# oi-taa/rag-fin

Hardware: AMD Instinct MI355X
Metric: queries/sec, brute-force cosine/IP top-10 over a 1,000,000 x 384-d fp16 corpus, batch=64 (recall@10 vs CPU oracle reported alongside) (higher is better)
Workload: dtype f16; 1 GPU; 1M x 384-d fp16 corpus, batch-64 queries, top-10; rows_per_gpu=1000000, rows_total=1000000, dim=384, batch=64, topk=10, batches_in_flight=4, collective=none

## Files before the change

rag_fin_amd/csrc/api.hip:

```cpp
#include "rf_internal.h"
#include <stdlib.h>
#include <string.h>

struct rf_arena {
  unsigned char* base;
  size_t off;
  template <class T>
  T* take(size_t count) {
    T* p = base ? (T*)(base + off) : nullptr;
    off = (off + count * sizeof(T) + 255) / 256 * 256;
    return p;
  }
};

static rf_workspace carve(rf_arena& a) {
  rf_workspace ws;
  ws.thr = a.take<float>(RF_QWIDE);
  ws.eps = a.take<float>(RF_QWIDE);
  ws.cand_cnt = a.take<uint32_t>((size_t)RF_QWIDE * RF_CAND_SHARDS);
  ws.pmax = a.take<float>((size_t)RF_QWIDE * RF_SAMPLE_WGS);
  ws.cand = a.take<uint2>((size_t)RF_QWIDE * RF_CAND_SHARDS * RF_SHARD_CAP);
  ws.fold = a.take<uint4>((size_t)RF_FOLD_WAVES * RF_QCHUNK);
  ws.rmask = a.take<unsigned long long>(RF_FOLD_WAVES);
  ws.rlist = a.take<uint32_t>(RF_FOLD_BLOCKS);
// ... 82 lines not shown
static int check_search_args(const char* fn, const rf_index_t* ix, const void* q, int B, int k,
                             const void* scores, const void* ids, const void* ws, size_t ws_bytes) {
  if (!ix || !q || !scores || !ids || !ws) {
    rf_set_error("%s: null argument", fn);
    return RF_ERR_INVALID;
  }
  if (B <= 0) {
    rf_set_error("%s: B = %d", fn, B);
    return RF_ERR_INVALID;
  }
  if (k <= 0 || k > RF_MAX_K) {
    rf_set_error("%s: k = %d outside 1..%d", fn, k, RF_MAX_K);
    return RF_ERR_UNSUPPORTED;
  }
  if ((((uintptr_t)q) & 15) || (((uintptr_t)ws) & 15)) {
    rf_set_error("%s: q / workspace must be 16-byte aligned", fn);
    return RF_ERR_INVALID;
  }
  if (ws_bytes < rf_search_workspace_bytes(nullptr)) {
    rf_set_error("%s: workspace %zu B < required %zu B", fn, ws_bytes,
                 rf_search_workspace_bytes(nullptr));
    return RF_ERR_CAPACITY;
  }
  return RF_OK;
}

static int check_sq8(const char* fn, const rf_index_t* ix, size_t ws_bytes) {
  if (!ix->sq8_tiles) {
    rf_set_error("%s: no SQ8 shadow attached (rf_index_attach_sq8)", fn);
    return RF_ERR_INVALID;
  }
  if (ws_bytes < rf_search_sq8_workspace_bytes(ix)) {
    rf_set_error("%s: workspace %zu B < required %zu B", fn, ws_bytes, rf_search_sq8_workspace_bytes(ix));
    return RF_ERR_CAPACITY;
  }
  return RF_OK;
}

static int check_filter_arg(const char* fn, const void* filter_dev) {
  if (!filter_dev || (((uintptr_t)filter_dev) & 15)) {
    rf_set_error("%s: filter buffer null or not 16-byte aligned", fn);
    return RF_ERR_INVALID;
  }
  return RF_OK;
}

__global__ void k_fill_empty(int n, int B, float* scores, int64_t* ids, double* exact,
                             uint32_t* flags) {
  const int i = blockIdx.x * blockDim.x + threadIdx.x;
  if (i < n) {
    scores[i] = -INFINITY;
    ids[i] = -1;
    if (exact) exact[i] = -INFINITY;
  }
  if (flags && i < B) flags[i] = 0u;
}

struct rf_out {
  float* scores;
  int64_t* ids;
  double* exact;
  uint32_t* flags;
};

static int fill_empty(int B, int k, const rf_out& o, hipStream_t st) {
  const int n = B * k;
  hipLaunchKernelGGL(k_fill_empty, dim3((n + 255) / 256), dim3(256), 0, st, n, B, o.scores, o.ids,
                     o.exact, o.flags);
  RF_HIP(hipGetLastError());
  return RF_OK;
}

static bool take_wide(const rf_index_t* ix, int left, int k) {
  return rf_wide_supported(ix) && left > RF_QCHUNK && ix->size > RF_SMALL_ROWS && k <= 16 &&
         ix->size >= (int64_t)k * 1024;
}

static int chunk_width(const rf_index_t* ix, int left, int k, bool widen, bool* wide) {
  *wide = widen && take_wide(ix, left, k);
  const int cap = *wide ? RF_QWIDE : RF_QCHUNK;
  return left < cap ? left : cap;
}

template <class T>
static T* at(T* p, size_t off) { return p ? p + off : nullptr; }

template <class F>
static int for_chunks(const rf_index_t* ix, const void* q_dev, int B, int k, size_t row, bool widen,
                      const rf_out& o, F&& body) {
  for (int q0 = 0; q0 < B;) {
    bool wide;
    const int nb = chunk_width(ix, B - q0, k, widen, &wide);
    const size_t r0 = (size_t)q0 * row;
    const int rc = body(q0, nb, wide, (const _Float16*)q_dev + (size_t)q0 * ix->dim,
                        rf_out{at(o.scores, r0), at(o.ids, r0), at(o.exact, r0), at(o.flags, (size_t)q0)});
    if (rc != RF_OK) return rc;
    q0 += nb;
  }
  return RF_OK;
}

struct rf_variant {
  const rf_filter_view* filt;
  const rf_sq8_ws* sq8;
  bool wide;
  const rf_band* band;
  const rf_after* after;
  const rf_multi* multi;
  bool coarse;
};

static int mark(hipEvent_t* ev, int* n, hipStream_t st) {
  if (ev) RF_HIP(hipEventRecord(ev[(*n)++], st));
  return RF_OK;
}

template <class F>
static int time_stages(int marks, float* stage_ms, F run) {
  hipEvent_t ev[7];
  for (int i = 0; i < marks; ++i) RF_HIP(hipEventCreate(&ev[i]));
  const int rc = run(ev);
  if (rc == RF_OK) {
    RF_HIP(hipEventSynchronize(ev[marks - 1]));
    for (int i = 0; i + 1 < marks; ++i) RF_HIP(hipEventElapsedTime(&stage_ms[i], ev[i], ev[i + 1]));
  }
  for (int i = 0; i < marks; ++i) (void)hipEventDestroy(ev[i]);
  return rc;
}

static int sweep(const rf_index_t* ix, const rf_variant& v, const _Float16* qc, int nb, int k, int64_t id_base,
                 const rf_workspace& ws, const rf_out& o, hipStream_t st, hipEvent_t* ev) {
  const int JB = nb <= 32 ? 1 : 2;
  int P = 0, n_ev = 0;
  rf_fold kept{};
  rf_fold* fold = (v.wide || v.sq8 || v.filt || v.band) ? nullptr : &kept;
  int rc = mark(ev, &n_ev, st);
  if (v.sq8) {
    if (rc == RF_OK) rc = rf_launch_sq8_queries(ix, qc, nb, *v.sq8, st);
    if (rc == RF_OK && !v.coarse) rc = mark(ev, &n_ev, st);
  }
  if (rc == RF_OK && ix->size > RF_SMALL_ROWS && v.band) rc = rf_launch_band_eps(ix, qc, nb, ws, st);
  if (rc == RF_OK && ix->size > RF_SMALL_ROWS)
    rc = v.wide ? rf_launch_wide_sample(ix, qc, nb, ws, &P, st)
                : rf_launch_sample(ix, qc, nb, JB, ws, &P, st, v.filt, fold, v.band, v.after, v.multi);
  if (rc == RF_OK) rc = mark(ev, &n_ev, st);
  if (rc == RF_OK) rc = rf_launch_threshold(ix, qc, nb, k, P, ws, st, fold, v.sq8, v.band);
  if (rc == RF_OK) rc = mark(ev, &n_ev, st);
  if (rc == RF_OK)
    rc = v.wide  ? rf_launch_wide_emit(ix, qc, nb, ws, st)
         : v.sq8 ? rf_launch_sq8_emit(ix, nb, JB, ws, *v.sq8, st)
                 : rf_launch_emit(ix, qc, nb, JB, ws, st, v.filt, fold, v.band, v.after, v.multi);
  if (v.sq8) {
    if (rc == RF_OK && !v.coarse) rc = mark(ev, &n_ev, st);
    if (rc == RF_OK) rc = rf_launch_shadow_refine(ix, qc, nb, k, ws, *v.sq8, st);
  }
  if (rc == RF_OK) rc = mark(ev, &n_ev, st);
  if (rc == RF_OK) rc = rf_launch_merge(ix, qc, nb, k, id_base, ws, o.scores, o.ids, o.exact, o.flags, st, v.band, v.after);
  if (rc == RF_OK) rc = mark(ev, &n_ev, st);
  return rc;
}

enum { RF_FP16 = 0, RF_SQ8 = 1, RF_SHADOW = 2 };
static int search_enqueue(const rf_index_t* ix, const void* q_dev, int B, int k, int64_t id_base, const rf_out& o,
                          void* workspace_dev, hipStream_t st, const rf_filter_view* filt, int sq8,
                          float* stage_ms = nullptr, const rf_band* band = nullptr,
                          const rf_after* after = nullptr, const rf_multi* multi = nullptr) {
  if (ix->size == 0) return fill_empty(B, k, o, st);
  rf_arena a{(unsigned char*)workspace_dev, 0};
  rf_workspace ws;
  const rf_sq8_ws sw = carve_sq8(a, &ws);
  const rf_sq8_ws* sq = sq8 != RF_FP16 && ix->size > RF_SMALL_ROWS ? &sw : nullptr;
  const bool coarse = sq8 == RF_SHADOW;
  const bool widen = !filt && !sq && !band;
  if (!stage_ms)
    return for_chunks(ix, q_dev, B, k, (size_t)k, widen, o,
                      [&](int q0, int nb, bool wide, const _Float16* qc, const rf_out& oc) {
                        const rf_after ac{after ? after->score + q0 : nullptr, after ? after->id + q0 : nullptr};
                        const rf_multi mc{multi ? multi->masks_t : nullptr, multi ? multi->qfilter + q0 : nullptr,
                                          multi ? multi->gp : 0u};
                        return sweep(ix, rf_variant{filt, sq, wide, band, after ? &ac : nullptr, multi ? &mc : nullptr, coarse},
                                     qc, nb, k, id_base, ws, oc, st, nullptr);
                      });
  bool wide;
  const int nb = chunk_width(ix, B, k, widen, &wide);
  return time_stages(sq && !coarse ? 7 : 5, stage_ms, [&](hipEvent_t* ev) {
    return sweep(ix, rf_variant{filt, sq, wide, band, after, multi, coarse}, (const _Float16*)q_dev, nb, k, id_base, ws,
                 o, st, ev);
  });
}

static int plain_chain(const rf_index_t* ix, int B) {
  return shadow_first(ix) && ix->size >= ix->shadow_min_rows && ix->size > RF_SMALL_ROWS && B <= RF_QCHUNK ? RF_SHADOW
                                                                                                          : RF_FP16;
}

extern "C" int rf_index_set_shadow_first(rf_index_t* ix, int64_t min_rows) {
  if (!ix) {
    rf_set_error("rf_index_set_shadow_first: null index");
    return RF_ERR_INVALID;
  }
  ix->shadow_min_rows = min_rows > 0 ? min_rows : 0;
  return RF_OK;
}

extern "C" int rf_search(const rf_index_t* ix, const void* q_dev, int B, int k, int64_t id_base,
                         float* scores_dev, int64_t* ids_dev, double* exact_dev,
                         uint32_t* flags_dev, void* workspace_dev, size_t workspace_bytes,
                         void* stream) {
  int rc = check_search_args("rf_search", ix, q_dev, B, k, scores_dev, ids_dev, workspace_dev,
                             workspace_bytes);
  if (rc == RF_OK && plain_chain(ix, B) == RF_SHADOW) rc = check_sq8("rf_search", ix, workspace_bytes);
  if (rc != RF_OK) return rc;
  return search_enqueue(ix, q_dev, B, k, id_base, rf_out{scores_dev, ids_dev, exact_dev, flags_dev}, workspace_dev,
                        (hipStream_t)stream, nullptr, plain_chain(ix, B));
}

extern "C" int rf_search_fp16(const rf_index_t* ix, const void* q_dev, int B, int k, int64_t id_base,
                              float* scores_dev, int64_t* ids_dev, double* exact_dev,
                              uint32_t* flags_dev, void* workspace_dev, size_t workspace_bytes,
                              void* stream) {
  int rc = check_search_args("rf_search_fp16", ix, q_dev, B, k, scores_dev, ids_dev, workspace_dev,
                             workspace_bytes);
  if (rc != RF_OK) return rc;
  return search_enqueue(ix, q_dev, B, k, id_base, rf_out{scores_dev, ids_dev, exact_dev, flags_dev}, workspace_dev,
                        (hipStream_t)stream, nullptr, RF_FP16);
}

extern "C" int rf_search_profile(const rf_index_t* ix, const void* q_dev, int B, int k,
                                 int64_t id_base, float* scores_dev, int64_t* ids_dev,
                                 double* exact_dev, uint32_t* flags_dev, void* workspace_dev,
                                 size_t workspace_bytes, void* stream, float* stage_ms_host) {
  int rc = check_search_args("rf_search_profile", ix, q_dev, B, k, scores_dev, ids_dev,
                             workspace_dev, workspace_bytes);
  if (rc == RF_OK && plain_chain(ix, B) == RF_SHADOW) rc = check_sq8("rf_search_profile", ix, workspace_bytes);
  if (rc != RF_OK) return rc;
  if (!stage_ms_host || ix->size == 0) {
    rf_set_error("rf_search_profile: null stage buffer or empty index");
    return RF_ERR_INVALID;
  }
  return search_enqueue(ix, q_dev, B, k, id_base, rf_out{scores_dev, ids_dev, exact_dev, flags_dev}, workspace_dev,
                        (hipStream_t)stream, nullptr, plain_chain(ix, B), stage_ms_host);
}

extern "C" int rf_search_sq8(const rf_index_t* ix, const void* q_dev, int B, int k, int64_t id_base,
                             float* scores_dev, int64_t* ids_dev, double* exact_dev, uint32_t* flags_dev,
                             void* workspace_dev, size_t workspace_bytes, void* stream) {
  int rc = check_search_args("rf_search_sq8", ix, q_dev, B, k, scores_dev, ids_dev, workspace_dev,
                             workspace_bytes);
  if (rc != RF_OK) return rc;
  rc = check_sq8("rf_search_sq8", ix, workspace_bytes);
  if (rc != RF_OK) return rc;
  return search_enqueue(ix, q_dev, B, k, id_base, rf_out{scores_dev, ids_dev, exact_dev, flags_dev}, workspace_dev,
                        (hipStream_t)stream, nullptr, RF_SQ8);
}

extern "C" int rf_search_sq8_profile(const rf_index_t* ix, const void* q_dev, int B, int k, int64_t id_base,
                                     float* scores_dev, int64_t* ids_dev, double* exact_dev, uint32_t* flags_dev,
                                     void* workspace_dev, size_t workspace_bytes, void* stream,
                                     float* stage_ms_host) {
  int rc = check_search_args("rf_search_sq8_profile", ix, q_dev, B, k, scores_dev, ids_dev, workspace_dev,
                             workspace_bytes);
  if (rc != RF_OK) return rc;
  rc = check_sq8("rf_search_sq8_profile", ix, workspace_bytes);
  if (rc != RF_OK) return rc;
  if (!stage_ms_host || ix->size <= RF_SMALL_ROWS) {
    rf_set_error("rf_search_sq8_profile: null stage buffer or a corpus of <= %d rows", RF_SMALL_ROWS);
    return RF_ERR_INVALID;
  }
  return search_enqueue(ix, q_dev, B, k, id_base, rf_out{scores_dev, ids_dev, exact_dev, flags_dev}, workspace_dev,
                        (hipStream_t)stream, nullptr, RF_SQ8, stage_ms_host);
}

extern "C" int rf_debug_scores_sq8(const rf_index_t* ix, const void* q_dev, int B, int64_t n, float* out_dev,
                                   float* delta_dev, void* workspace_dev, size_t workspace_bytes, void* stream) {
  if (!ix || !q_dev || !out_dev || !workspace_dev || B <= 0 || n <= 0 || n > ix->size) {
    rf_set_error("rf_debug_scores_sq8: bad argument");
    return RF_ERR_INVALID;
  }
  int rc = check_sq8("rf_debug_scores_sq8", ix, workspace_bytes);
  if (rc != RF_OK) return rc;
  hipStream_t st = (hipStream_t)stream;
  rf_arena a{(unsigned char*)workspace_dev, 0};
  const rf_sq8_ws sw = carve_sq8(a, nullptr);
  return for_chunks(ix, q_dev, B, 0, (size_t)n, false, rf_out{out_dev, nullptr, nullptr, nullptr},
                    [&](int q0, int nb, bool, const _Float16* qc, const rf_out& oc) {
                      const int rc = rf_launch_sq8_queries(ix, qc, nb, sw, st);
                      return rc != RF_OK ? rc : rf_launch_sq8_debug(ix, nb, n, sw, oc.scores, at(delta_dev, (size_t)q0), st);
                    });
}

static int exhaustive_impl(const char* fn, const rf_index_t* ix, const void* q_dev, int B, int k,
                           int64_t id_base, float* scores_dev, int64_t* ids_dev, double* exact_dev,
                           const double* after_s, const int64_t* after_r, void* workspace_dev,
                           size_t workspace_bytes, void* stream, const uint32_t* mask = nullptr,
                           const rf_band* band = nullptr) {
  int rc = check_search_args(fn, ix, q_dev, B, k, scores_dev, ids_dev, workspace_dev, workspace_bytes);
  if (rc != RF_OK) return rc;
  hipStream_t st = (hipStream_t)stream;
  const rf_out o{scores_dev, ids_dev, exact_dev, nullptr};
  if (ix->size == 0) return fill_empty(B, k, o, st);
  rf_arena a{(unsigned char*)workspace_dev, 0};
  const rf_workspace ws = carve(a);
  return for_chunks(ix, q_dev, B, k, (size_t)k, false, o,
                    [&](int q0, int nb, bool, const _Float16* qc, const rf_out& oc) {
                      return rf_launch_exhaustive(ix, qc, nb, k, id_base, ws, oc.scores, oc.ids, oc.exact,
                                                  at(after_s, (size_t)q0), at(after_r, (size_t)q0), st, mask, band);
                    });
// ... 339 lines not shown
```

rag_fin_amd/csrc/rf_internal.h:

```cpp
#pragma once
#include <hip/hip_runtime.h>
#include <stdint.h>
#include <stddef.h>
#include <atomic>
#include <mutex>
#include <vector>
#include "../../include/ragfin.h"

#define RF_BLOCK_ROWS 32
#define RF_FRAG_BYTES 1024

__host__ __device__ inline size_t rf_chunk_index(int64_t row, int chunk, int KS) {
  const int64_t b = row >> 5;
  const int r = (int)(row & 31);
  return ((size_t)b * KS + (chunk >> 1)) * 64 + (size_t)((chunk & 1) * 32 + r);
}

struct rf_index {
  int dim;
  int KS;
  int device;
  int64_t capacity;
  int64_t size;
  uint4* tiles;
  uint32_t* max_norm2;
  size_t storage_bytes;
  int num_cus;
  uint4* sq8_tiles;
  float* sq8_scale;
  float* sq8_err;
  uint32_t* sq8_max;
  int64_t shadow_min_rows;
};

#define RF_KNOBS(X)                                                                                                  \
  X(ring24, 8, 6, 24)                \
  X(emit_wgs_per_cu, 0, 0, 4)                                  \
  X(sample_bpw, 2, 1, 8)                                                                 \
  X(sq8_ring12, 6, 4, 12)         \
  X(sample_fold, 1, 0, 1)         \
  X(fold_dbg, 0, 0, 3)            \
  X(wide_sample_pairs, 4, 1, 8)                            \
  X(wide_dbg, 0, 0, 63)           \
  X(wide_ne, 0, 0, 112)             \
  X(linear_dma, 1, 0, 3)          \
  X(linear_small, 1, 0, 1)             \
  X(encode_graph, 1, 0, 1)                               \
  X(linear_dbg, 0, 0, 63)                                   \
  X(debug_epi, 0, 0, 5)           \
  X(one_query, 1, 0, 1)           \
  X(post_block, 1, 0, 1)          \
  X(post_qkv, 1, 0, 1)                      \
  X(post_dbg, 0, 0, 511)
#ifdef RF_EXPERIMENTS
#define RF_KNOB_DECL(name, dflt, lo, hi) extern int rf_knob_##name;
#else
#define RF_KNOB_DECL(name, dflt, lo, hi) static constexpr int rf_knob_##name = dflt;
#endif
RF_KNOBS(RF_KNOB_DECL)
#undef RF_KNOB_DECL
#ifdef RF_EXPERIMENTS
extern int rf_tuning_generation;
extern void* rf_debug_buffer;
#else
static constexpr int rf_tuning_generation = 0;
static constexpr void* rf_debug_buffer = nullptr;
#endif

#define RF_MAX_DEVICES 64
struct rf_lds_attr {
  std::atomic<uint32_t> bytes[RF_MAX_DEVICES];
};
static inline hipError_t rf_ensure_lds(rf_lds_attr& a, const void* fn, size_t lds) {
  int dev = 0;
  hipError_t e = hipGetDevice(&dev);
  if (e != hipSuccess) return e;
  if (dev < 0 || dev >= RF_MAX_DEVICES) return hipErrorInvalidDevice;
  if (a.bytes[dev].load(std::memory_order_relaxed) >= lds) return hipSuccess;
  e = hipFuncSetAttribute(fn, hipFuncAttributeMaxDynamicSharedMemorySize, (int)lds);
  if (e == hipSuccess) a.bytes[dev].store((uint32_t)lds, std::memory_order_relaxed);
  return e;
}

#define RF_QWIDE 256
#define RF_CAND_CAP 8192
#define RF_CAND_SHARDS 8
#define RF_SHARD_CAP 2048
#define RF_SMALL_ROWS 8192
#define RF_SAMPLE_WGS 256
#define RF_RESCORE_CAP 256
#define RF_FOLD_WAVES (RF_SAMPLE_WGS * 8)
#define RF_FOLD_BLOCKS (RF_FOLD_WAVES * 8)

struct rf_workspace {
  float* thr;
  float* eps;
  uint32_t* cand_cnt;
  float* pmax;
  uint2* cand;
  uint4* fold;
  unsigned long long* rmask;
  uint32_t* rlist;
  uint32_t* rcnt;
  double* ex_score;
  int64_t* ex_row;
};
#define RF_EX_WGS 256

void rf_set_error(const char* fmt, ...);
#define RF_HIP(call)                                                              \
  do {                                                                            \
    hipError_t e_ = (call);                                                       \
    if (e_ != hipSuccess) {                                                       \
      rf_set_error("%s failed: %s (%s:%d)", #call, hipGetErrorString(e_), __FILE__, \
                   __LINE__);                                                     \
      return RF_ERR_HIP;                                                          \
    }                                                                             \
  } while (0)

void rf_launch_tile_rows(const void* rows, uint4* tiles, int64_t first_row, int64_t n, int KS,
                         hipStream_t st);
#define RF_FILTER_HDR_WORDS 4
#define RF_FILTER_MAX_TILES 1024
struct rf_filter_view {
  const uint32_t* hdr;
  const uint32_t* mask;
  const uint32_t* blocks;
};
size_t rf_filter_layout(int64_t n_rows, size_t* mask_off, size_t* blocks_off, size_t* tiles_off);
rf_filter_view rf_filter_carve(const void* filter, int64_t n_rows);
struct rf_multi {
  const uint32_t* masks_t;
  const int32_t* qfilter;
  uint32_t gp;
};
uint32_t rf_multi_columns(int n_filters);
size_t rf_multi_layout(int64_t n_rows, int n_filters, size_t* masks_off);

struct rf_fold {
  uint32_t n_samp;
  uint32_t bstride;
  uint32_t W;
};
struct rf_band {
  double lo, hi;
};
struct rf_after {
  const double* score;
  const int64_t* id;
};
int rf_launch_sample(const rf_index* ix, const void* q, int B, int JB, const rf_workspace& ws,
                     int* P_out, hipStream_t st, const rf_filter_view* filt = nullptr,
                     rf_fold* fold = nullptr, const rf_band* band = nullptr, const rf_after* after = nullptr,
                     const rf_multi* multi = nullptr);
int rf_launch_emit(const rf_index* ix, const void* q, int B, int JB, const rf_workspace& ws,
                   hipStream_t st, const rf_filter_view* filt = nullptr, const rf_fold* fold = nullptr,
                   const rf_band* band = nullptr, const rf_after* after = nullptr,
                   const rf_multi* multi = nullptr);
static inline int rf_waves_per_wg(int KS) { return KS >= 48 ? 8 : 4; }
static inline int rf_emit_grid(const rf_index* ix, int wgs_per_cu) {
  const int WAVES = rf_waves_per_wg(ix->KS);
  const uint32_t nblk = (uint32_t)((ix->size + 31) / 32);
  int grid = ix->num_cus * (wgs_per_cu > 0 ? wgs_per_cu : (ix->KS >= 48 ? 1 : 2));
  const uint32_t need = (nblk + WAVES - 1) / WAVES;
  if ((uint32_t)grid > need) grid = (int)need;
  return grid < 1 ? 1 : grid;
}
int rf_launch_debug_scores(const rf_index* ix, const void* q, int B, int64_t n, float* out,
                           hipStream_t st);
int rf_scan_supported_dim(int dim);
int rf_wide_supported(const rf_index* ix);
int rf_launch_wide_sample(const rf_index* ix, const void* q, int B, const rf_workspace& ws, int* P_out,
                          hipStream_t st);
int rf_launch_wide_emit(const rf_index* ix, const void* q, int B, const rf_workspace& ws, hipStream_t st);
struct rf_sq8_ws {
  int8_t* q8;
  float* tq;
  float* nq;
  float* fq;
};
int rf_sq8_quantize_rows(rf_index* ix, int64_t row0, int64_t row1, hipStream_t st);
int rf_launch_sq8_queries(const rf_index* ix, const void* q, int B, const rf_sq8_ws& sw, hipStream_t st);
int rf_launch_sq8_emit(const rf_index* ix, int B, int JB, const rf_workspace& ws, const rf_sq8_ws& sw,
                       hipStream_t st);
int rf_launch_sq8_debug(const rf_index* ix, int B, int64_t n, const rf_sq8_ws& sw, float* out, float* delta,
                        hipStream_t st);
int rf_launch_shadow_refine(const rf_index* ix, const void* q, int B, int k, const rf_workspace& ws,
                            const rf_sq8_ws& sw, hipStream_t st);
int rf_launch_threshold(const rf_index* ix, const void* q, int B, int k, int P,
                        const rf_workspace& ws, hipStream_t st, const rf_fold* fold = nullptr,
                        const rf_sq8_ws* sq8 = nullptr, const rf_band* band = nullptr);
int rf_launch_band_eps(const rf_index* ix, const void* q, int B, const rf_workspace& ws, hipStream_t st);
int rf_launch_merge(const rf_index* ix, const void* q, int B, int k, int64_t id_base,
                    const rf_workspace& ws, float* scores, int64_t* ids, double* exact,
// ... 77 lines not shown
```

rag_fin_amd/csrc/sq8.hip:

```cpp
#include "rf_internal.h"
#include "scan_common.h"
#include "sq8.h"

typedef int32_t i32x4 __attribute__((ext_vector_type(4)));
typedef int32_t i32x16 __attribute__((ext_vector_type(16)));

static inline int64_t sq8_blocks(int64_t rows) { return (rows + RF_BLOCK_ROWS - 1) / RF_BLOCK_ROWS; }

__device__ __forceinline__ double wave_sum_xor(double v) {
  for (int o = 32; o > 0; o >>= 1) v += __shfl_xor(v, o);
  return v;
}
__device__ __forceinline__ float sq8_code(float x, float s) {
  return s > 0.f ? fminf(fmaxf(rintf(x / s), -127.f), 127.f) : 0.f;
}

__global__ void __launch_bounds__(256) k_sq8_rows(const uint4* __restrict__ tiles, int KS, int64_t row0,
                                                  int64_t row1, uint2* __restrict__ t8,
                                                  float* __restrict__ scale, float* __restrict__ err,
                                                  uint32_t* __restrict__ mx) {
  const int lane = threadIdx.x & 63;
  const int64_t wave = ((int64_t)blockIdx.x * blockDim.x + threadIdx.x) >> 6;
  const int64_t nwaves = ((int64_t)gridDim.x * blockDim.x) >> 6;
  const int chunks = 2 * KS;
  const int KS8 = KS / 2;
  float nbest = 0.f, ebest = 0.f;
  for (int64_t row = row0 + wave; row < row1; row += nwaves) {
    half8 v[2];
    float m = 0.f;
#pragma unroll
    for (int j = 0; j < 2; ++j) {
      const int c = lane + 64 * j;
      v[j] = __builtin_bit_cast(half8, c < chunks ? tiles[rf_chunk_index(row, c, KS)] : make_uint4(0, 0, 0, 0));
#pragma unroll
      for (int e = 0; e < 8; ++e) m = fmaxf(m, fabsf((float)v[j][e]));
    }
    m = wave_max_xor(m);
    const float s = m / 127.f;
    double r2 = 0.0, n2 = 0.0;
    const int64_t b = row >> 5;
    const int r = (int)(row & 31);
#pragma unroll
    for (int j = 0; j < 2; ++j) {
      const int c = lane + 64 * j;
      uint32_t w[2] = {0u, 0u};
#pragma unroll
      for (int e = 0; e < 8; ++e) {
        const float x = (float)v[j][e];
        const float cq = sq8_code(x, s);
        w[e >> 2] |= ((uint32_t)(int32_t)cq & 0xFFu) << (8 * (e & 3));
        const double y = (double)s * (double)cq;
        const double d = (double)x - y;
        r2 = fma(d, d, r2);
        n2 = fma(y, y, n2);
      }
      if (c < chunks) {
        const int u = c >> 1;
        const size_t idx = ((size_t)b * KS8 + (u >> 1)) * 64 + (size_t)((u & 1) * 32 + r);
        t8[idx * 2 + (c & 1)] = make_uint2(w[0], w[1]);
      }
    }
    r2 = wave_sum_xor(r2);
    n2 = wave_sum_xor(n2);
    const float e = rf_sqrt_up(r2);
    if (lane == 0) {
      const size_t slot = (size_t)b * 32 + rf_sq8_slot(r);
      scale[slot] = s;
      err[slot] = e;
    }
    nbest = fmaxf(nbest, rf_sqrt_up(n2));
    ebest = fmaxf(ebest, e);
  }
  if (lane == 0) {
    if (nbest > 0.f) atomicMax(&mx[0], __builtin_bit_cast(uint32_t, nbest));
    if (ebest > 0.f) atomicMax(&mx[1], __builtin_bit_cast(uint32_t, ebest));
  }
}

__global__ void __launch_bounds__(64) k_sq8_queries(const _Float16* __restrict__ q, int B, int dim,
                                                    int8_t* __restrict__ q8, float* __restrict__ tq,
                                                    float* __restrict__ nq, float* __restrict__ fq) {
  const int qi = blockIdx.x;
  const int lane = threadIdx.x;
  if (qi >= B) {
    if (lane == 0) tq[qi] = nq[qi] = fq[qi] = 0.f;
    return;
  }
  const _Float16* row = q + (size_t)qi * dim;
  float m = 0.f;
  for (int d = lane; d < dim; d += 64) m = fmaxf(m, fabsf((float)row[d]));
  m = wave_max_xor(m);
  const float t = m / 127.f;
  double n2 = 0.0, f2 = 0.0;
  for (int d = lane; d < dim; d += 64) {
    const float x = (float)row[d];
    const float cq = sq8_code(x, t);
    q8[(size_t)qi * dim + d] = (int8_t)(int32_t)cq;
    const double dd = (double)x - (double)t * (double)cq;
    n2 = fma((double)x, (double)x, n2);
    f2 = fma(dd, dd, f2);
  }
  n2 = wave_sum_xor(n2);
  f2 = wave_sum_xor(f2);
  if (lane == 0) {
    tq[qi] = t;
    nq[qi] = rf_sqrt_up(n2);
    fq[qi] = rf_sqrt_up(f2);
  }
}

struct Sq8Params {
  const uint4* corpus;
  const float* scale;
  const float* err;
  const int8_t* q8;
  const float* tq;
  const float* nq;
  int B, dim;
  uint32_t n_rows, n_work;
  const float* thr;
  uint32_t* cand_cnt;
  uint2* cand;
  uint32_t cap;
};

struct Sq8ListFull {
  unsigned long long* sat;
  __device__ __forceinline__ void operator()(uint32_t q) const { atomicOr(sat, 1ull << q); }
};

struct Sq8Meta {
  float4 s[4], e[4];
};
__device__ __forceinline__ void load_meta(Sq8Meta& m, const Sq8Params& p, uint32_t b, int h) {
  const float4* sp = (const float4*)(p.scale + (size_t)b * 32 + h * 16);
  const float4* ep = (const float4*)(p.err + (size_t)b * 32 + h * 16);
#pragma unroll
  for (int j = 0; j < 4; ++j) {
    m.s[j] = sp[j];
    m.e[j] = ep[j];
  }
}
__device__ __forceinline__ float f4_at(const float4 (&v)[4], int i) {
  const float4 x = v[i >> 2];
  return (i & 3) == 0 ? x.x : (i & 3) == 1 ? x.y : (i & 3) == 2 ? x.z : x.w;
}

template <int KS8, int R, int JB, bool LAST>
__device__ __forceinline__ void sq8_step(u32x4 (&ring)[R], Sq8Meta& meta, uint32_t b, uint32_t bn,
                                         const u32x4* smemQ, int lane, const float (&th)[JB],
                                         const float (&tq)[JB], const float (&nq)[JB], EmitState& es,
                                         const Sq8Params& p, unsigned long long* sat) {
  static_assert(KS8 % R == 0, "ring must divide the block");
  asm volatile("" ::: "memory");
  const int h = lane >> 5;
  const uint4* cur = p.corpus + (size_t)b * (KS8 * 64) + lane;
  const uint4* nxt = p.corpus + (size_t)bn * (KS8 * 64) + lane;
  Sq8Meta next;
  if (!LAST) load_meta(next, p, bn, h);
  i32x16 acc[JB];
#pragma unroll
  for (int jb = 0; jb < JB; ++jb)
#pragma unroll
    for (int i = 0; i < 16; ++i) acc[jb][i] = 0;
#pragma unroll
  for (int kk = 0; kk < KS8; ++kk) {
    const i32x4 a = __builtin_bit_cast(i32x4, ring[kk % R]);
#pragma unroll
    for (int jb = 0; jb < JB; ++jb) {
      const i32x4 bq = __builtin_bit_cast(i32x4, smemQ[(jb * KS8 + kk) * 64 + lane]);
      acc[jb] = __builtin_amdgcn_mfma_i32_32x32x32_i8(a, bq, acc[jb], 0, 0, 0);
    }
    if (kk + R < KS8) {
      ring[kk % R] = ld_frag(cur + (kk + R) * 64);
    } else if (!LAST) {
      ring[kk % R] = ld_frag(nxt + (kk + R - KS8) * 64);
    }
  }
  const uint32_t row0 = b * 32u;
  const uint32_t lim = p.n_rows - row0;
  const unsigned long long full = *(volatile unsigned long long*)sat;
  f32x16 sc[JB];
  uint32_t bits = 0u;
#pragma unroll
  for (int jb = 0; jb < JB; ++jb)
#pragma unroll
    for (int i = 0; i < 16; ++i) {
      const float a = __fmul_rn(__fmul_rn(tq[jb], f4_at(meta.s, i)), (float)acc[jb][i]);
      sc[jb][i] = a;
      const bool ok = (a + nq[jb] * f4_at(meta.e, i) >= th[jb]) && (acc_row(i, h) < lim) &&
                      ((full >> (jb * 32 + (lane & 31))) & 1ull) == 0ull;
      bits |= ok ? (1u << (jb * 16 + i)) : 0u;
    }
  if (__ballot(bits != 0u) != 0ull) emit_append<JB>(sc, bits, row0, lane, es, [&] { emit_flush(es, p, lane, Sq8ListFull{sat}); });
  if (!LAST) meta = next;
}

template <int KS8, int R, int JB>
__global__ void __launch_bounds__(256, 2) k_sq8_emit(Sq8Params p) {
  constexpr int WAVES = 4;
  extern __shared__ __attribute__((aligned(16))) unsigned char smem_raw[];
  __shared__ unsigned long long sat;
  u32x4* smemQ = (u32x4*)smem_raw;
  unsigned char* tail = smem_raw + (size_t)JB * KS8 * RF_FRAG_BYTES;
  const int tid = threadIdx.x;
  const int lane = tid & 63;
  const int wave = __builtin_amdgcn_readfirstlane(tid >> 6);
  const int h = lane >> 5;

  float th[JB], tq[JB], nq[JB];
#pragma unroll
  for (int jb = 0; jb < JB; ++jb) {
    const int qi = jb * 32 + (lane & 31);
    th[jb] = p.thr[qi];
    tq[jb] = p.tq[qi];
    nq[jb] = p.nq[qi];
  }
  EmitState es = emit_state((uint32_t*)tail, wave, WAVES, SCAP);
  const uint32_t W = gridDim.x * WAVES;
  const uint32_t gw = blockIdx.x * WAVES + wave;
  u32x4 ring[R];
  Sq8Meta meta;
  if (gw < p.n_work) {
    const uint4* src = p.corpus + (size_t)gw * (KS8 * 64) + lane;
#pragma unroll
    for (int s = 0; s < R; ++s) ring[s] = ld_frag(src + s * 64);
    load_meta(meta, p, gw, h);
  }
  if (tid == 0) sat = 0ull;
  stage_queries<KS8, JB, WAVES>(smemQ, p.q8, p.B);
  __syncthreads();
  const uint32_t cnt = (p.n_work > gw) ? (p.n_work - gw + W - 1) / W : 0u;
  if (cnt > 0) {
    uint32_t b = gw;
    for (uint32_t i = 0; i + 1 < cnt; ++i, b += W)
      sq8_step<KS8, R, JB, false>(ring, meta, b, b + W, smemQ, lane, th, tq, nq, es, p, &sat);
    sq8_step<KS8, R, JB, true>(ring, meta, b, b, smemQ, lane, th, tq, nq, es, p, &sat);
  }
  if (es.cnt > 0) emit_flush(es, p, lane, Sq8ListFull{&sat});
}

__global__ void __launch_bounds__(64) k_sq8_debug(const uint4* __restrict__ t8, const float* __restrict__ scale,
                                                  int KS8, const int8_t* __restrict__ q8, const float* __restrict__ tq,
                                                  const float* __restrict__ nq, const float* __restrict__ fq,
                                                  const uint32_t* __restrict__ mx, int B, int dim, uint32_t n,
                                                  float* __restrict__ out, float* __restrict__ delta) {
  const int lane = threadIdx.x;
  const int h = lane >> 5;
  const uint32_t b = blockIdx.x;
  const int qi = blockIdx.y * 32 + (lane & 31);
  i32x16 acc;
#pragma unroll
  for (int i = 0; i < 16; ++i) acc[i] = 0;
  for (int kk = 0; kk < KS8; ++kk) {
    const uint4 av = t8[((size_t)b * KS8 + kk) * 64 + lane];
    uint4 bv = make_uint4(0, 0, 0, 0);
    if (qi < B) bv = *(const uint4*)(q8 + (size_t)qi * dim + kk * 32 + h * 16);
    acc = __builtin_amdgcn_mfma_i32_32x32x32_i8(__builtin_bit_cast(i32x4, av), __builtin_bit_cast(i32x4, bv), acc,
                                                0, 0, 0);
  }
  if (qi >= B) return;
#pragma unroll
  for (int i = 0; i < 16; ++i) {
    const uint32_t row = b * 32u + acc_row(i, h);
    if (row < n)
      out[(size_t)qi * n + row] = __fmul_rn(__fmul_rn(tq[qi], scale[(size_t)b * 32 + h * 16 + i]), (float)acc[i]);
  }
  if (b == 0 && h == 0 && delta)
    delta[qi] = rf_sq8_delta(nq[qi], fq[qi], __builtin_bit_cast(float, mx[0]), __builtin_bit_cast(float, mx[1]));
}

__global__ void k_sq8_get_rows(const uint4* __restrict__ t8, const float* __restrict__ scale,
                               const float* __restrict__ err, const int64_t* __restrict__ rows, int64_t n, int KS8,
                               int64_t size, uint4* __restrict__ out, float* __restrict__ s_out,
                               float* __restrict__ e_out) {
  const int units = 2 * KS8;
  const int64_t total = n * units;
  int64_t i = (int64_t)blockIdx.x * blockDim.x + threadIdx.x;
  const int64_t stride = (int64_t)gridDim.x * blockDim.x;
  for (; i < total; i += stride) {
    const int64_t j = i / units;
    const int u = (int)(i % units);
    const int64_t row = rows[j];
    const bool ok = row >= 0 && row < size;
    const int64_t b = ok ? row >> 5 : 0;
    const int r = ok ? (int)(row & 31) : 0;
    out[i] = ok ? t8[((size_t)b * KS8 + (u >> 1)) * 64 + (u & 1) * 32 + r] : make_uint4(0, 0, 0, 0);
    if (u == 0) {
      s_out[j] = ok ? scale[(size_t)b * 32 + rf_sq8_slot(r)] : 0.f;
      e_out[j] = ok ? err[(size_t)b * 32 + rf_sq8_slot(r)] : 0.f;
    }
  }
}

static inline int grid_for(int64_t work_items, int block) {
  int64_t g = (work_items + block - 1) / block;
  if (g < 1) g = 1;
  if (g > 2048) g = 2048;
  return (int)g;
}

extern "C" size_t rf_sq8_storage_bytes(int dim, int64_t capacity_rows) {
  if (dim <= 0 || dim % 32 != 0 || !rf_scan_supported_dim(dim) || capacity_rows <= 0) return 0;
  const size_t blocks = (size_t)sq8_blocks(capacity_rows);
  return blocks * ((size_t)(dim / 32) * RF_FRAG_BYTES + 2 * 32 * sizeof(float)) + 256;
}

int rf_sq8_quantize_rows(rf_index* ix, int64_t row0, int64_t row1, hipStream_t st) {
  const int64_t end = sq8_blocks(row1) * RF_BLOCK_ROWS;
  if (end <= row0) return RF_OK;
  hipLaunchKernelGGL(k_sq8_rows, dim3(grid_for((end - row0) * 64, 256)), dim3(256), 0, st, ix->tiles, ix->KS,
                     row0, end, (uint2*)ix->sq8_tiles, ix->sq8_scale, ix->sq8_err, ix->sq8_max);
  RF_HIP(hipGetLastError());
  return RF_OK;
}

extern "C" int rf_index_attach_sq8(rf_index_t* ix, void* storage_dev, size_t storage_bytes, void* stream) {
  if (!ix || !storage_dev) {
    rf_set_error("rf_index_attach_sq8: null argument");
    return RF_ERR_INVALID;
  }
  if (ix->dim % 32 != 0) {
    rf_set_error("rf_index_attach_sq8: SQ8 needs dim %% 32 == 0 (dim %d)", ix->dim);
    return RF_ERR_UNSUPPORTED;
  }
  const size_t need = rf_sq8_storage_bytes(ix->dim, ix->capacity);
  if (storage_bytes < need) {
    rf_set_error("rf_index_attach_sq8: storage %zu B < required %zu B", storage_bytes, need);
    return RF_ERR_CAPACITY;
  }
  if (((uintptr_t)storage_dev & 15) != 0) {
    rf_set_error("rf_index_attach_sq8: storage not 16-byte aligned");
    return RF_ERR_INVALID;
  }
  const size_t blocks = (size_t)sq8_blocks(ix->capacity);
  unsigned char* base = (unsigned char*)storage_dev;
  ix->sq8_tiles = (uint4*)base;
  ix->sq8_scale = (float*)(base + blocks * (ix->dim / 32) * RF_FRAG_BYTES);
  ix->sq8_err = ix->sq8_scale + blocks * 32;
  ix->sq8_max = (uint32_t*)(ix->sq8_err + blocks * 32);
  hipStream_t st = (hipStream_t)stream;
  RF_HIP(hipMemsetAsync(ix->sq8_max, 0, 256, st));
  if (ix->size > 0) return rf_sq8_quantize_rows(ix, 0, ix->size, st);
  return RF_OK;
}

extern "C" int rf_index_detach_sq8(rf_index_t* ix) {
  if (!ix) {
    rf_set_error("rf_index_detach_sq8: null index");
    return RF_ERR_INVALID;
  }
  ix->sq8_tiles = nullptr;
  ix->sq8_scale = nullptr;
  ix->sq8_err = nullptr;
  ix->sq8_max = nullptr;
  return RF_OK;
}

extern "C" int rf_index_get_rows_sq8(const rf_index_t* ix, const int64_t* rows_dev, int64_t n, void* out_dev,
                                     float* scales_dev, float* err_dev, void* stream) {
  if (!ix || !rows_dev || !out_dev || !scales_dev || !err_dev || n < 0) {
    rf_set_error("rf_index_get_rows_sq8: bad argument");
    return RF_ERR_INVALID;
  }
  if (!ix->sq8_tiles) {
    rf_set_error("rf_index_get_rows_sq8: no SQ8 shadow attached");
    return RF_ERR_INVALID;
  }
  if (((uintptr_t)out_dev & 15) != 0) {
    rf_set_error("rf_index_get_rows_sq8: out not 16-byte aligned");
    return RF_ERR_INVALID;
  }
  if (n == 0) return RF_OK;
  const int KS8 = ix->dim / 32;
  hipLaunchKernelGGL(k_sq8_get_rows, dim3(grid_for(n * KS8 * 2, 256)), dim3(256), 0, (hipStream_t)stream,
                     ix->sq8_tiles, ix->sq8_scale, ix->sq8_err, rows_dev, n, KS8, ix->size, (uint4*)out_dev,
                     scales_dev, err_dev);
  RF_HIP(hipGetLastError());
  return RF_OK;
}

int rf_launch_sq8_queries(const rf_index* ix, const void* q, int B, const rf_sq8_ws& sw, hipStream_t st) {
  hipLaunchKernelGGL(k_sq8_queries, dim3(RF_QCHUNK), dim3(64), 0, st, (const _Float16*)q, B, ix->dim, sw.q8, sw.tq,
                     sw.nq, sw.fq);
  RF_HIP(hipGetLastError());
  return RF_OK;
}

int rf_launch_sq8_debug(const rf_index* ix, int B, int64_t n, const rf_sq8_ws& sw, float* out, float* delta,
                        hipStream_t st) {
  const dim3 grid((unsigned)((n + 31) / 32), (B + 31) / 32);
  hipLaunchKernelGGL(k_sq8_debug, grid, dim3(64), 0, st, ix->sq8_tiles, ix->sq8_scale, ix->dim / 32, sw.q8, sw.tq,
                     sw.nq, sw.fq, ix->sq8_max, B, ix->dim, (uint32_t)n, out, delta);
  RF_HIP(hipGetLastError());
  return RF_OK;
}

template <int KS8, int R, int JB>
static int launch_sq8(const Sq8Params& p, int grid, hipStream_t st) {
  const size_t lds = (size_t)JB * KS8 * RF_FRAG_BYTES + (size_t)3 * 4 * SCAP * 4;
  static rf_lds_attr attr;
  RF_HIP(rf_ensure_lds(attr, (const void*)k_sq8_emit<KS8, R, JB>, lds));
  hipLaunchKernelGGL((k_sq8_emit<KS8, R, JB>), dim3(grid), dim3(256), lds, st, p);
  RF_HIP(hipGetLastError());
  return RF_OK;
}

int rf_launch_sq8_emit(const rf_index* ix, int B, int JB, const rf_workspace& ws, const rf_sq8_ws& sw,
                       hipStream_t st) {
  const uint32_t nblk = (uint32_t)((ix->size + 31) / 32);
  int grid = ix->num_cus * 2;
  const uint32_t need = (nblk + 3) / 4;
  if ((uint32_t)grid > need) grid = (int)need;
  if (grid < 1) grid = 1;
  Sq8Params p{};
  p.corpus = ix->sq8_tiles;
  p.scale = ix->sq8_scale;
  p.err = ix->sq8_err;
  p.q8 = sw.q8;
  p.tq = sw.tq;
  p.nq = sw.nq;
  p.B = B;
  p.dim = ix->dim;
  p.n_rows = (uint32_t)ix->size;
  p.n_work = nblk;
  p.thr = ws.thr;
  p.cand_cnt = ws.cand_cnt;
  p.cand = ws.cand;
  p.cap = RF_SHARD_CAP;
#define RF_SQ8(ks8, r) \
  case ks8:            \
    return JB == 1 ? launch_sq8<ks8, r, 1>(p, grid, st) : launch_sq8<ks8, r, 2>(p, grid, st);
#ifdef RF_EXPERIMENTS
  if (ix->dim / 32 == 12 && rf_knob_sq8_ring12 == 12)
    return JB == 1 ? launch_sq8<12, 12, 1>(p, grid, st) : launch_sq8<12, 12, 2>(p, grid, st);
  if (ix->dim / 32 == 12 && rf_knob_sq8_ring12 == 4)
    return JB == 1 ? launch_sq8<12, 4, 1>(p, grid, st) : launch_sq8<12, 4, 2>(p, grid, st);
#endif
  switch (ix->dim / 32) {
    RF_SQ8(2, 2) RF_SQ8(4, 4) RF_SQ8(8, 8) RF_SQ8(12, 6) RF_SQ8(16, 8) RF_SQ8(24, 12) RF_SQ8(32, 8)
    default:
      break;
  }
#undef RF_SQ8
  rf_set_error("no SQ8 emit kernel for dim %d", ix->dim);
  return RF_ERR_UNSUPPORTED;
}
```

Baseline: 793,600 queries/s.

## Hand-schedule SQ8 emit scan with explicit vmcnt waits and nontemporal loads

Rewrites the SQ8 emit inner loop to issue corpus fragment loads through inline asm with the nt hint and wait on exact vmcnt counts, instead of relying on compiler-inserted waits. Query operands from LDS are prefetched one k-step ahead, and the saturation bitmap uses an LDS-scoped relaxed atomic. The threshold test is restructured to fold the saturated-query check into the threshold and simplify the row-limit check. It also changes the ring depth for dim 768 at JB=2 and adds a debug knob bit that skips shadow refine. Hand-counted vmcnt values are fragile and could be wrong if the compiler emits other memory ops.

Result: no change. 798,200 queries/s, median of 6 (+0.6%).

```diff
diff --git a/rag_fin_amd/csrc/api.hip b/rag_fin_amd/csrc/api.hip
--- a/rag_fin_amd/csrc/api.hip
+++ b/rag_fin_amd/csrc/api.hip
@@ -258,7 +258,7 @@
                  : rf_launch_emit(ix, qc, nb, JB, ws, st, v.filt, fold, v.band, v.after, v.multi);
   if (v.sq8) {
     if (rc == RF_OK && !v.coarse) rc = mark(ev, &n_ev, st);
-    if (rc == RF_OK) rc = rf_launch_shadow_refine(ix, qc, nb, k, ws, *v.sq8, st);
+    if (rc == RF_OK && !(rf_knob_fold_dbg & 4)) rc = rf_launch_shadow_refine(ix, qc, nb, k, ws, *v.sq8, st);
   }
   if (rc == RF_OK) rc = mark(ev, &n_ev, st);
   if (rc == RF_OK) rc = rf_launch_merge(ix, qc, nb, k, id_base, ws, o.scores, o.ids, o.exact, o.flags, st, v.band, v.after);
diff --git a/rag_fin_amd/csrc/rf_internal.h b/rag_fin_amd/csrc/rf_internal.h
--- a/rag_fin_amd/csrc/rf_internal.h
+++ b/rag_fin_amd/csrc/rf_internal.h
@@ -39,7 +39,7 @@
   X(sample_bpw, 2, 1, 8)                                                                 \
   X(sq8_ring12, 6, 4, 12)         \
   X(sample_fold, 1, 0, 1)         \
-  X(fold_dbg, 0, 0, 3)            \
+  X(fold_dbg, 0, 0, 7)            \
   X(wide_sample_pairs, 4, 1, 8)                            \
   X(wide_dbg, 0, 0, 63)           \
   X(wide_ne, 0, 0, 112)             \
diff --git a/rag_fin_amd/csrc/sq8.hip b/rag_fin_amd/csrc/sq8.hip
--- a/rag_fin_amd/csrc/sq8.hip
+++ b/rag_fin_amd/csrc/sq8.hip
@@ -1,5 +1,6 @@
 #include "rf_internal.h"
 #include "scan_common.h"
+#include "lds_ring.h"
 #include "sq8.h"
 
 typedef int32_t i32x4 __attribute__((ext_vector_type(4)));
@@ -124,76 +125,116 @@
   uint32_t cap;
 };
 
+typedef __attribute__((address_space(3))) unsigned long long* sq8_sat_ptr;
 struct Sq8ListFull {
-  unsigned long long* sat;
-  __device__ __forceinline__ void operator()(uint32_t q) const { atomicOr(sat, 1ull << q); }
+  sq8_sat_ptr sat;
+  __device__ __forceinline__ void operator()(uint32_t q) const {
+    __hip_atomic_fetch_or(sat, 1ull << q, __ATOMIC_RELAXED, __HIP_MEMORY_SCOPE_WORKGROUP);
+  }
 };
 
+typedef float f32x4 __attribute__((ext_vector_type(4)));
 struct Sq8Meta {
-  float4 s[4], e[4];
+  f32x4 s[4], e[4];
 };
-__device__ __forceinline__ void load_meta(Sq8Meta& m, const Sq8Params& p, uint32_t b, int h) {
-  const float4* sp = (const float4*)(p.scale + (size_t)b * 32 + h * 16);
-  const float4* ep = (const float4*)(p.err + (size_t)b * 32 + h * 16);
-#pragma unroll
-  for (int j = 0; j < 4; ++j) {
-    m.s[j] = sp[j];
-    m.e[j] = ep[j];
-  }
-}
-__device__ __forceinline__ float f4_at(const float4 (&v)[4], int i) {
-  const float4 x = v[i >> 2];
-  return (i & 3) == 0 ? x.x : (i & 3) == 1 ? x.y : (i & 3) == 2 ? x.z : x.w;
+__device__ __forceinline__ float f4_at(const f32x4 (&v)[4], int i) { return v[i >> 2][i & 3]; }
+
+template <int OFF>
+__device__ __forceinline__ void sq8_ld_nt(u32x4& d, uint32_t voff, const void* base) {
+  asm volatile("global_load_dwordx4 %0, %1, %2 offset:%3 nt" : "+v"(d) : "v"(voff), "s"(base), "n"(OFF));
+}
+template <int OFF>
+__device__ __forceinline__ void sq8_ld(f32x4& d, uint32_t voff, const void* base) {
+  asm volatile("global_load_dwordx4 %0, %1, %2 offset:%3" : "=v"(d) : "v"(voff), "s"(base), "n"(OFF));
+}
+template <int F>
+__device__ __forceinline__ void sq8_ld_frag(u32x4& d, uint32_t voff, const unsigned char* blk) {
+  sq8_ld_nt<(F & 3) * 1024>(d, voff, blk + (F & ~3) * 1024);
+}
+__device__ __forceinline__ void sq8_ld_meta(Sq8Meta& m, const Sq8Params& p, uint32_t b, uint32_t moff) {
+  const float* sp = p.scale + (size_t)b * 32;
+  const float* ep = p.err + (size_t)b * 32;
+  sq8_ld<0>(m.s[0], moff, sp); sq8_ld<16>(m.s[1], moff, sp); sq8_ld<32>(m.s[2], moff, sp); sq8_ld<48>(m.s[3], moff, sp);
+  sq8_ld<0>(m.e[0], moff, ep); sq8_ld<16>(m.e[1], moff, ep); sq8_ld<32>(m.e[2], moff, ep); sq8_ld<48>(m.e[3], moff, ep);
+}
+constexpr int SQ8_META_LOADS = 8;
+template <int N>
+__device__ __forceinline__ void sq8_wait_frag(u32x4& d) {
+  asm volatile("s_waitcnt vmcnt(%1)" : "+v"(d) : "n"(N));
+}
+template <int N>
+__device__ __forceinline__ void sq8_wait_meta(Sq8Meta& m) {
+  asm volatile("s_waitcnt vmcnt(%8)" : "+v"(m.s[0]), "+v"(m.s[1]), "+v"(m.s[2]), "+v"(m.s[3]),
+               "+v"(m.e[0]), "+v"(m.e[1]), "+v"(m.e[2]), "+v"(m.e[3]) : "n"(N));
 }
 
 template <int KS8, int R, int JB, bool LAST>
 __device__ __forceinline__ void sq8_step(u32x4 (&ring)[R], Sq8Meta& meta, uint32_t b, uint32_t bn,
                                          const u32x4* smemQ, int lane, const float (&th)[JB],
                                          const float (&tq)[JB], const float (&nq)[JB], EmitState& es,
-                                         const Sq8Params& p, unsigned long long* sat) {
+                                         const Sq8Params& p, sq8_sat_ptr sat) {
   static_assert(KS8 % R == 0, "ring must divide the block");
   asm volatile("" ::: "memory");
   const int h = lane >> 5;
-  const uint4* cur = p.corpus + (size_t)b * (KS8 * 64) + lane;
-  const uint4* nxt = p.corpus + (size_t)bn * (KS8 * 64) + lane;
+  const uint32_t voff = (uint32_t)lane * 16u, moff = (uint32_t)h * 64u;
+  const unsigned char* cur = (const unsigned char*)p.corpus + (size_t)b * (KS8 * 1024);
+  const unsigned char* nxt = (const unsigned char*)p.corpus + (size_t)bn * (KS8 * 1024);
+  const unsigned long long full = *(volatile __attribute__((address_space(3))) unsigned long long*)sat;
   Sq8Meta next;
-  if (!LAST) load_meta(next, p, bn, h);
+  if (!LAST) sq8_ld_meta(next, p, bn, moff);
   i32x16 acc[JB];
 #pragma unroll
   for (int jb = 0; jb < JB; ++jb)
 #pragma unroll
     for (int i = 0; i < 16; ++i) acc[jb][i] = 0;
-#pragma unroll
-  for (int kk = 0; kk < KS8; ++kk) {
+  i32x4 bq[JB];
+#pragma unroll
+  for (int jb = 0; jb < JB; ++jb) bq[jb] = __builtin_bit_cast(i32x4, smemQ[(jb * KS8) * 64 + lane]);
+  static_for<0, KS8>([&](auto Kc) __attribute__((always_inline)) {
+    constexpr int kk = decltype(Kc)::value;
+    constexpr int frags = (LAST ? (kk + R < KS8 ? kk + R : KS8) : kk + R) - 1 - kk;
+    sq8_wait_frag<frags + ((!LAST && kk < R) ? SQ8_META_LOADS : 0)>(ring[kk % R]);
     const i32x4 a = __builtin_bit_cast(i32x4, ring[kk % R]);
-#pragma unroll
-    for (int jb = 0; jb < JB; ++jb) {
-      const i32x4 bq = __builtin_bit_cast(i32x4, smemQ[(jb * KS8 + kk) * 64 + lane]);
-      acc[jb] = __builtin_amdgcn_mfma_i32_32x32x32_i8(a, bq, acc[jb], 0, 0, 0);
-    }
-    if (kk + R < KS8) {
-      ring[kk % R] = ld_frag(cur + (kk + R) * 64);
-    } else if (!LAST) {
-      ring[kk % R] = ld_frag(nxt + (kk + R - KS8) * 64);
-    }
-  }
+    i32x4 bqn[JB];
+    if constexpr (kk + 1 < KS8) {
+#pragma unroll
+      for (int jb = 0; jb < JB; ++jb) bqn[jb] = __builtin_bit_cast(i32x4, smemQ[(jb * KS8 + kk + 1) * 64 + lane]);
+    }
+#pragma unroll
+    for (int jb = 0; jb < JB; ++jb) acc[jb] = __builtin_amdgcn_mfma_i32_32x32x32_i8(a, bq[jb], acc[jb], 0, 0, 0);
+    __builtin_amdgcn_sched_barrier(0);
+    if constexpr (kk + R < KS8) sq8_ld_frag<kk + R>(ring[kk % R], voff, cur);
+    else if constexpr (!LAST) sq8_ld_frag<kk + R - KS8>(ring[kk % R], voff, nxt);
+    if constexpr (kk + 1 < KS8) {
+#pragma unroll
+      for (int jb = 0; jb < JB; ++jb) bq[jb] = bqn[jb];
+    }
+  });
   const uint32_t row0 = b * 32u;
   const uint32_t lim = p.n_rows - row0;
-  const unsigned long long full = *(volatile unsigned long long*)sat;
+  const int lim_h = (int)(lim < 32u ? lim : 32u) - 4 * h;
   f32x16 sc[JB];
   uint32_t bits = 0u;
 #pragma unroll
-  for (int jb = 0; jb < JB; ++jb)
-#pragma unroll
-    for (int i = 0; i < 16; ++i) {
+  for (int jb = JB - 1; jb >= 0; --jb) {
+    const float thj = ((full >> (jb * 32 + (lane & 31))) & 1ull) != 0ull ? __builtin_inff() : th[jb];
+#pragma unroll
+    for (int i = 15; i >= 0; --i) {
       const float a = __fmul_rn(__fmul_rn(tq[jb], f4_at(meta.s, i)), (float)acc[jb][i]);
       sc[jb][i] = a;
-      const bool ok = (a + nq[jb] * f4_at(meta.e, i) >= th[jb]) && (acc_row(i, h) < lim) &&
-                      ((full >> (jb * 32 + (lane & 31))) & 1ull) == 0ull;
-      bits |= ok ? (1u << (jb * 16 + i)) : 0u;
-    }
-  if (__ballot(bits != 0u) != 0ull) emit_append<JB>(sc, bits, row0, lane, es, [&] { emit_flush(es, p, lane, Sq8ListFull{sat}); });
-  if (!LAST) meta = next;
+      const bool ok = (a + nq[jb] * f4_at(meta.e, i) >= thj) && ((int)acc_row(i, 0) < lim_h);
+      bits = (bits << 1) | (ok ? 1u : 0u);
+    }
+  }
+  if (__ballot(bits != 0u) != 0ull)
+    emit_append<JB>(sc, bits, row0, lane, es, [&] {
+      emit_flush(es, p, lane, Sq8ListFull{sat});
+      asm volatile("s_waitcnt vmcnt(0)" ::: "memory");
+    });
+  if (!LAST) {
+    sq8_wait_meta<R>(next);
+    meta = next;
+  }
 }
 
 template <int KS8, int R, int JB>
@@ -201,6 +242,7 @@
   constexpr int WAVES = 4;
   extern __shared__ __attribute__((aligned(16))) unsigned char smem_raw[];
   __shared__ unsigned long long sat;
+  const sq8_sat_ptr satp = (sq8_sat_ptr)&sat;
   u32x4* smemQ = (u32x4*)smem_raw;
   unsigned char* tail = smem_raw + (size_t)JB * KS8 * RF_FRAG_BYTES;
   const int tid = threadIdx.x;
@@ -222,22 +264,25 @@
   u32x4 ring[R];
   Sq8Meta meta;
   if (gw < p.n_work) {
-    const uint4* src = p.corpus + (size_t)gw * (KS8 * 64) + lane;
-#pragma unroll
-    for (int s = 0; s < R; ++s) ring[s] = ld_frag(src + s * 64);
-    load_meta(meta, p, gw, h);
+    sq8_ld_meta(meta, p, gw, (uint32_t)h * 64u);
+    static_for<0, R>([&](auto Sc) __attribute__((always_inline)) {
+      sq8_ld_frag<decltype(Sc)::value>(ring[decltype(Sc)::value], (uint32_t)lane * 16u,
+                                       (const unsigned char*)p.corpus + (size_t)gw * (KS8 * 1024));
+    });
   }
   if (tid == 0) sat = 0ull;
   stage_queries<KS8, JB, WAVES>(smemQ, p.q8, p.B);
   __syncthreads();
   const uint32_t cnt = (p.n_work > gw) ? (p.n_work - gw + W - 1) / W : 0u;
   if (cnt > 0) {
+    sq8_wait_meta<0>(meta);
+    static_for<0, R>([&](auto Sc) __attribute__((always_inline)) { sq8_wait_frag<0>(ring[decltype(Sc)::value]); });
     uint32_t b = gw;
     for (uint32_t i = 0; i + 1 < cnt; ++i, b += W)
-      sq8_step<KS8, R, JB, false>(ring, meta, b, b + W, smemQ, lane, th, tq, nq, es, p, &sat);
-    sq8_step<KS8, R, JB, true>(ring, meta, b, b, smemQ, lane, th, tq, nq, es, p, &sat);
-  }
-  if (es.cnt > 0) emit_flush(es, p, lane, Sq8ListFull{&sat});
+      sq8_step<KS8, R, JB, false>(ring, meta, b, b + W, smemQ, lane, th, tq, nq, es, p, satp);
+    sq8_step<KS8, R, JB, true>(ring, meta, b, b, smemQ, lane, th, tq, nq, es, p, satp);
+  }
+  if (es.cnt > 0) emit_flush(es, p, lane, Sq8ListFull{satp});
 }
 
 __global__ void __launch_bounds__(64) k_sq8_debug(const uint4* __restrict__ t8, const float* __restrict__ scale,
@@ -428,9 +473,10 @@
   p.cand_cnt = ws.cand_cnt;
   p.cand = ws.cand;
   p.cap = RF_SHARD_CAP;
-#define RF_SQ8(ks8, r) \
-  case ks8:            \
-    return JB == 1 ? launch_sq8<ks8, r, 1>(p, grid, st) : launch_sq8<ks8, r, 2>(p, grid, st);
+#define RF_SQ8(ks8, r) RF_SQ8_2(ks8, r, r)
+#define RF_SQ8_2(ks8, r1, r2) \
+  case ks8:                   \
+    return JB == 1 ? launch_sq8<ks8, r1, 1>(p, grid, st) : launch_sq8<ks8, r2, 2>(p, grid, st);
 #ifdef RF_EXPERIMENTS
   if (ix->dim / 32 == 12 && rf_knob_sq8_ring12 == 12)
     return JB == 1 ? launch_sq8<12, 12, 1>(p, grid, st) : launch_sq8<12, 12, 2>(p, grid, st);
@@ -438,11 +484,12 @@
     return JB == 1 ? launch_sq8<12, 4, 1>(p, grid, st) : launch_sq8<12, 4, 2>(p, grid, st);
 #endif
   switch (ix->dim / 32) {
-    RF_SQ8(2, 2) RF_SQ8(4, 4) RF_SQ8(8, 8) RF_SQ8(12, 6) RF_SQ8(16, 8) RF_SQ8(24, 12) RF_SQ8(32, 8)
+    RF_SQ8(2, 2) RF_SQ8(4, 4) RF_SQ8(8, 8) RF_SQ8(12, 6) RF_SQ8(16, 8) RF_SQ8_2(24, 12, 8) RF_SQ8(32, 8)
     default:
       break;
   }
 #undef RF_SQ8
+#undef RF_SQ8_2
   rf_set_error("no SQ8 emit kernel for dim %d", ix->dim);
   return RF_ERR_UNSUPPORTED;
 }
```
